# secup/ProjectUltra

Hardware: AMD Instinct MI355X
Metric: OFDM-1024 16QAM R3/4 frames decoded/sec (higher is better)
Workload: dtype f32

## Files before the change

projectultra_amd/csrc/demod_kernel.h:

```cpp
#ifndef ULTRA_DEMOD_KERNEL_H
#define ULTRA_DEMOD_KERNEL_H

#include <hip/hip_runtime.h>
#include <utility>
#include "device_types.h"
#include "pinned_math.h"
#include "phase_table.h"

namespace ultra_hip {
namespace dev {

constexpr int kWave = 64;
constexpr int kPhaseCap = 48;

__device__ __forceinline__ c32 mk(float re, float im) { c32 r; r.re = re; r.im = im; return r; }
__device__ __forceinline__ c32 cadd(c32 a, c32 b) { return mk(a.re + b.re, a.im + b.im); }
__device__ __forceinline__ c32 csub(c32 a, c32 b) { return mk(a.re - b.re, a.im - b.im); }
__device__ __forceinline__ c32 cconj(c32 a) { return mk(a.re, -a.im); }
__device__ __forceinline__ c32 cmul(c32 x, c32 y) {
    float ac = x.re * y.re, bd = x.im * y.im, ad = x.re * y.im, bc = x.im * y.re;
    return mk(ac - bd, ad + bc);
}
__device__ __forceinline__ c32 cdiv(c32 x, c32 y) {
    double a = x.re, b = x.im, c = y.re, d = y.im;
// ... 1346 lines not shown
    const LaneConst lc = lane_constants(D);
    for (int frame = blockIdx.x; frame < n_frames; frame += gridDim.x) {
        float* st = state + (size_t)frame * kStFloats;
        Track tr;
        load_track(st, tr);
        const bool presynced_loop = D.presynced && !synced_loop;
        const bool scalar_pilot_half = D.n_pilot == 0 && !presynced_loop;
        const bool compact = compact_pilot_state(D);
        if (!compact) sh.H[lane] = reinterpret_cast<const c32*>(st + kStH)[lane];
        else if (lane < D.n_pilot) sh.H[lc.pilot_slot] = reinterpret_cast<const c32*>(st + kStHp)[lane];
        c32 dprev = D.differential ? reinterpret_cast<const c32*>(st + kStDprev)[lane] : mk(1.0f, 0.0f);
        const bool adaptive = D.adaptive_eq != 0 && !D.differential;
        AdaptiveEq ad;
        ad.w = mk(1.0f, 0.0f); ad.P = 1.0f;
        if (adaptive) { ad.w = reinterpret_cast<const c32*>(st + kStLms)[lane]; ad.P = st[kStRlsP + lane]; }
        wave_sync();
        float dprev_abs = -1.0f;
        const bool tc_is_fixed = D.differential && D.n_pilot == 0 && n_sym_batch > 1;
        c32 tc0 = mk(1.0f, 0.0f);
        if (tc_is_fixed) tc0 = cexpj_bounded(timing_phase_of(lc.data_k, tr.timing, D.log2_fft));
        for (int ds = 0; ds < n_sym_batch; ++ds) {
            const c32* fq = fq_all + ((size_t)ds * n_frames + frame) * (2 * D.fq_half);
            if (scalar_pilot_half) { tr.ppc = mk(1.0f, 0.0f); tr.has_prev = 0; tr.snr_symbol_count++; }
            if (!presynced_loop || D.n_pilot != 0) {
                finish_channel_estimate(sh, D, lc, tr);
                if (adaptive && tr.snr_symbol_count - 1 < 3 && lane < D.n_data) ad.w = sh.H[lc.data_slot];
            }
            equalize_demap<MOD>(sh, D, lc, tr, dprev, fq,
                                llr + (size_t)frame * llr_stride + (size_t)(data_sym + ds) * D.llrs_per_symbol,
                                &dprev_abs, tc_is_fixed ? &tc0 : nullptr, nullptr, adaptive ? &ad : nullptr,
                                EQ ? eq_out + (size_t)frame * eq_stride + (size_t)ds * kMaxCarriers : nullptr);
            wave_sync();
        }
        if (!compact) reinterpret_cast<c32*>(st + kStH)[lane] = sh.H[lane];
        else if (lane < ((D.n_pilot + 15) & ~15))
            reinterpret_cast<c32*>(st + kStHp)[lane] = (lane < D.n_pilot) ? sh.H[lc.pilot_slot] : mk(0.0f, 0.0f);
        if (D.differential) reinterpret_cast<c32*>(st + kStDprev)[lane] = dprev;
        if (adaptive) { reinterpret_cast<c32*>(st + kStLms)[lane] = ad.w; st[kStRlsP + lane] = ad.P; }
        if (lane == 0) {
            st[st_ppc_re] = tr.ppc.re; st[st_ppc_im] = tr.ppc.im;
            st[st_flags] = (float)(tr.cpc_init | (tr.has_prev << 1) | (tr.has_dprev << 2));
            if (scalar_pilot_half) st[st_count] = (float)tr.snr_symbol_count;
            if (state_out) {
                float* so = state_out + (size_t)frame * ULTRA_HIP_STATE_FLOATS;
                so[ULTRA_HIP_STATE_FREQ_OFFSET_HZ] = tr.freq_offset_hz;
                so[ULTRA_HIP_STATE_NOISE_VARIANCE] = tr.noise_variance;
                so[ULTRA_HIP_STATE_SNR_LINEAR] = tr.snr_linear;
                so[ULTRA_HIP_STATE_TIMING_OFFSET] = tr.timing;
                so[ULTRA_HIP_STATE_CFO_PHASE] = tr.cfo_phase;
                so[ULTRA_HIP_STATE_MIXER_PHASE] = D.mixer_phase_end;
                so[ULTRA_HIP_STATE_SYMBOLS] = (float)tr.snr_symbol_count;
                so[ULTRA_HIP_STATE_RESERVED] = 0.0f;
            }
        }
        wave_sync();
    }
}

template <int MOD>
__global__ __launch_bounds__(kWave, 6) void track_diff_pair_kernel(
    const DemodConst* __restrict__ Dp, int n_frames, int data_sym, float* __restrict__ state,
    const c32* __restrict__ fq_all, float* __restrict__ llr, size_t llr_stride, float* __restrict__ state_out,
    int n_sym_batch) {
    static_assert(MOD == ULTRA_MOD_DBPSK || MOD == ULTRA_MOD_DQPSK || MOD == ULTRA_MOD_D8PSK, "differential layouts");
    constexpr int kBits = (MOD == ULTRA_MOD_DBPSK) ? 1 : (MOD == ULTRA_MOD_DQPSK) ? 2 : 3;
    const DemodConst& D = *Dp;
    const int lane = threadIdx.x, g = lane >> 5, sub = lane & 31;
    const bool is_data = sub < D.n_data;
    const int dsl = is_data ? D.data_slot[sub] : 0;
    const int data_fq = fq_index(D, D.bin[dsl]), data_k = D.k_of[dsl];
    const unsigned long long half_mask = g ? 0xffffffff00000000ull : 0x00000000ffffffffull;
    const int n_pairs = (n_frames + 1) / 2;
    for (int pair = blockIdx.x; pair < n_pairs; pair += gridDim.x) {
        const bool live = 2 * pair + g < n_frames;
        const int frame = live ? 2 * pair + g : n_frames - 1;
        float* st = state + (size_t)frame * kStFloats;
        Track tr;
        load_track(st, tr);
        c32 H = reinterpret_cast<const c32*>(st + kStH)[dsl];
        c32 dprev = reinterpret_cast<const c32*>(st + kStDprev)[sub];
        if (!tr.has_dprev) dprev = mk(1.0f, 0.0f);
        float prev_abs = cabs_(dprev);
        const c32 tc = cexpj_bounded(timing_phase_of(data_k, tr.timing, D.log2_fft));
        for (int ds = 0; ds < n_sym_batch; ++ds) {
            const c32* fq = fq_all + ((size_t)ds * n_frames + frame) * (2 * D.fq_half);
            tr.ppc = mk(1.0f, 0.0f); tr.has_prev = 0; tr.snr_symbol_count++;
            c32 eq = mk(0.0f, 0.0f);
            float nv = 100.0f;
            if (is_data) {
                const c32 received = fq[data_fq];
                const float h_power = cnorm(H);
                if (h_power > 1e-6f) {
                    const c32 t = cdivf(cmul(received, cconj(H)), h_power);
                    eq = cmul(cmul(t, tr.ppc), tc);
                    nv = tr.noise_variance / h_power;
                } else {
                    eq = cmul(cmul(received, tr.ppc), tc);
                    nv = 100.0f;
                }
                nv = fmax_std(1e-6f, fmin_std(100.0f, nv));
            }
            const float eq_abs = cabs_(eq);
            if (is_data) {
                float out[kBits];
                demap_carrier<MOD>(eq, dprev, nv * D.ce_margin, out, eq_abs, prev_abs);
                if (live) {
                    float* dst = llr + (size_t)frame * llr_stride + (size_t)(data_sym + ds) * D.llrs_per_symbol + sub * kBits;
#pragma unroll
                    for (int b = 0; b < kBits; ++b) dst[b] = out[b];
                }
                dprev = eq;
                prev_abs = eq_abs;
            }
            if ((MOD == ULTRA_MOD_DQPSK || MOD == ULTRA_MOD_D8PSK) && tr.snr_symbol_count >= 1) {
                bool strong = false;
                if (is_data) {
                    const float a = eq_abs;
                    strong = (a * a) > 0.1f;
                    if (strong) H = cmul(H, mk(1.0f, -0.0f));
                }
                const int valid = __popcll(__ballot(strong) & half_mask);
                if (valid >= 5) {
                    c32 p = cmul(cscale(tr.ppc, 1.0f), mk(1.0f, -0.0f));
                    const float mag = cabs_(p);
                    if (mag > 0.01f) p = cdivf(p, mag);
                    tr.ppc = p;
                }
            }
            tr.has_dprev = 1;
        }
        if (live && is_data) {
            reinterpret_cast<c32*>(st + kStH)[dsl] = H;
            reinterpret_cast<c32*>(st + kStDprev)[sub] = dprev;
        }
        if (live && sub == 0) {
            st[st_ppc_re] = tr.ppc.re; st[st_ppc_im] = tr.ppc.im;
            st[st_flags] = (float)(tr.cpc_init | (tr.has_prev << 1) | (tr.has_dprev << 2));
            st[st_count] = (float)tr.snr_symbol_count;
            if (state_out) {
                float* so = state_out + (size_t)frame * ULTRA_HIP_STATE_FLOATS;
                so[ULTRA_HIP_STATE_FREQ_OFFSET_HZ] = tr.freq_offset_hz;
                so[ULTRA_HIP_STATE_NOISE_VARIANCE] = tr.noise_variance;
                so[ULTRA_HIP_STATE_SNR_LINEAR] = tr.snr_linear;
                so[ULTRA_HIP_STATE_TIMING_OFFSET] = tr.timing;
                so[ULTRA_HIP_STATE_CFO_PHASE] = tr.cfo_phase;
                so[ULTRA_HIP_STATE_MIXER_PHASE] = D.mixer_phase_end;
                so[ULTRA_HIP_STATE_SYMBOLS] = (float)tr.snr_symbol_count;
                so[ULTRA_HIP_STATE_RESERVED] = 0.0f;
            }
        }
    }
}

template <int MOD>
__global__ __launch_bounds__(kWave, 6) void track_all_kernel(const DemodConst* __restrict__ Dp, int n_frames, int sym0, int n_sym_batch,
                                                             const float* __restrict__ trk_rec, const c32* __restrict__ fq_all,
                                                             float* __restrict__ llr, size_t llr_stride, float* __restrict__ state_out,
                                                             const float* __restrict__ state) {
    __shared__ TrackShared sh;
    const DemodConst& D = *Dp;
    const int lane = threadIdx.x;
    const LaneConst lc = lane_constants(D);
    const int total = n_frames * n_sym_batch;
    const int rec_floats = trk_rec_floats(D.n_pilot), rec_hp = trk_rec_hp(D.n_pilot);
    const int rec_mask = (D.n_pilot <= kTrkRecCompactPilots) ? 1 : 7;
    float nx_rec = 0.0f;
    c32 nx_hp = mk(0.0f, 0.0f), nx_fq = mk(0.0f, 0.0f);
    auto request = [&](int w) {
        const float* rec = trk_rec + (size_t)w * rec_floats;
        nx_rec = rec[lane & rec_mask];
        if (lane < D.n_pilot) nx_hp = reinterpret_cast<const c32*>(rec + rec_hp)[lane];
        if (lane < D.n_data) nx_fq = fq_all[(size_t)w * (2 * D.fq_half) + lc.data_fq];
    };
    if ((int)blockIdx.x < total) request((int)blockIdx.x);
    for (int w = blockIdx.x; w < total; w += gridDim.x) {
        const int frame = w % n_frames, ds = w / n_frames;
        Track tr;
        const float my_rec = nx_rec;
        const c32 my_hp = nx_hp, my_fq = nx_fq;
        if (w + (int)gridDim.x < total) request(w + (int)gridDim.x);
        tr.noise_variance = __int_as_float(__builtin_amdgcn_readlane(__float_as_int(my_rec), tk_noise));
        tr.timing = __int_as_float(__builtin_amdgcn_readlane(__float_as_int(my_rec), tk_timing));
        tr.ppc = mk(1.0f, 0.0f); tr.cpc = mk(1.0f, 0.0f);
        tr.cpc_init = 1; tr.has_prev = 1; tr.has_dprev = 0; tr.snr_symbol_count = 0; tr.symbols_since_sync = 0;
        if (lane < D.n_pilot) sh.H[lc.pilot_slot] = my_hp;
        c32 dprev = mk(1.0f, 0.0f);
        wave_sync();
        finish_channel_estimate(sh, D, lc, tr);
        equalize_demap<MOD>(sh, D, lc, tr, dprev, fq_all + (size_t)w * (2 * D.fq_half),
                            llr + (size_t)frame * llr_stride + (size_t)(sym0 + ds) * D.llrs_per_symbol, nullptr, nullptr, &my_fq);
        if (state_out && lane == 0 && ds == n_sym_batch - 1) {
            const float* st = state + (size_t)frame * kStFloats;
            float* so = state_out + (size_t)frame * ULTRA_HIP_STATE_FLOATS;
            so[ULTRA_HIP_STATE_FREQ_OFFSET_HZ] = st[st_cfo];
            so[ULTRA_HIP_STATE_NOISE_VARIANCE] = st[st_noise];
            so[ULTRA_HIP_STATE_SNR_LINEAR] = st[st_snr];
            so[ULTRA_HIP_STATE_TIMING_OFFSET] = st[st_timing];
            so[ULTRA_HIP_STATE_CFO_PHASE] = st[st_cfo_phase];
            so[ULTRA_HIP_STATE_MIXER_PHASE] = D.mixer_phase_end;
            so[ULTRA_HIP_STATE_SYMBOLS] = st[st_count];
            so[ULTRA_HIP_STATE_RESERVED] = 0.0f;
        }
        wave_sync();
    }
}

}
}
#endif
```

projectultra_amd/csrc/ultra_hip.hip:

```cpp
#include <hip/hip_runtime.h>

#include <dlfcn.h>
#include <cmath>
#include <cstdio>
#include <cstdlib>
#include <cstring>
#include <new>
#include <atomic>
#include <chrono>
#include <vector>

#include "../../include/ultra_hip.h"
#include "device_types.h"
#include "host_tables.h"
#include "demod_kernel.h"
#include "ldpc_kernel.h"
#include "ldpc_screen_kernel.h"
#include "ldpc_totals_kernel.h"
#include "acquire_kernel.h"
#include "stimulus_kernel.h"
#include "chirp_kernel.h"
#include "frame_kernel.h"

using namespace ultra_hip;
// ... 155 lines not shown
}
int ensure_list_workspace(ultra_hip_ctx* ctx, size_t n_cw) {
    if (ctx->ws_list_cw >= n_cw) return ULTRA_HIP_OK;
    if (ctx->d_ws_list) { UH_HIP(uh_stream_sync(ctx->stream)); (void)hipFree(ctx->d_ws_list); ctx->d_ws_list = nullptr; }
    ctx->ws_list_cw = 0;
    UH_HIP(hipMalloc(&ctx->d_ws_list, n_cw * sizeof(unsigned)));
    ctx->ws_list_cw = n_cw;
    return ULTRA_HIP_OK;
}
int ensure_llr_workspace(ultra_hip_ctx* ctx, size_t n_frames) {
    if (ctx->ws_llr_frames >= n_frames) return ULTRA_HIP_OK;
    if (ctx->d_ws_llr) { UH_HIP(uh_stream_sync(ctx->stream)); (void)hipFree(ctx->d_ws_llr); ctx->d_ws_llr = nullptr; }
    ctx->ws_llr_frames = 0;
    UH_HIP(hipMalloc(&ctx->d_ws_llr, n_frames * (size_t)ctx->geo.llrs_per_frame * sizeof(float)));
    ctx->ws_llr_frames = n_frames;
    return ULTRA_HIP_OK;
}

int launch_demod(ultra_hip_ctx* ctx, const float* d_audio, size_t frame_stride, const float* d_cfo_hz,
                 const float* d_cfo_phase, size_t n_frames, float* d_llr, size_t llr_stride, float* d_state,
                 const unsigned* d_frame_offset = nullptr, int sym_begin = 0, int sym_count = -1, c32* d_eq = nullptr) {
    if (n_frames == 0) return ULTRA_HIP_OK;
    const DemodConst& D = ctx->h_demod;
    const int s_begin = sym_begin, s_end = (sym_count < 0) ? D.n_train + D.n_data_sym : sym_begin + sym_count;
    if (s_begin < 0 || s_end > D.n_train + D.n_data_sym || s_end <= s_begin) return ULTRA_HIP_ERR_INVALID_ARG;
    if (s_begin > 0 && ctx->ws_demod_frames < n_frames) return ULTRA_HIP_ERR_INVALID_ARG;
    const int start_mode = (s_begin == 0 && sym_count >= 0) ? ctx->stream_start_mode : ULTRA_STREAM_START_FRESH;
    const float* start_timing = (start_mode == ULTRA_STREAM_START_TIMING) ? ctx->stream_start_timing : nullptr;
    if (s_begin == 0 && sym_count >= 0) { ctx->stream_start_mode = ULTRA_STREAM_START_FRESH; ctx->stream_start_timing = nullptr; }
    if (start_mode == ULTRA_STREAM_START_SYNC && (ctx->ws_demod_frames < n_frames || D.presynced)) return ULTRA_HIP_ERR_INVALID_ARG;
    const bool cfo_given = (s_begin == 0) ? (d_cfo_hz != nullptr || start_mode != ULTRA_STREAM_START_FRESH) : ctx->stream_cfo_given;
    if (s_begin == 0) ctx->stream_cfo_given = cfo_given;
    { const int rc_ws = ensure_demod_workspace(ctx, n_frames); if (rc_ws != ULTRA_HIP_OK) return rc_ws; }
    auto mix_grid = [&](size_t items) {
        size_t per_cu = ctx->mix_wg_per_cu > 0 ? (size_t)ctx->mix_wg_per_cu
                                               : std::min<size_t>(128, std::max<size_t>(24, items / ((size_t)ctx->cu_count * 24)));
        return (unsigned)std::min(items, (size_t)ctx->cu_count * per_cu);
    };
    const unsigned grid_fft = mix_grid(n_frames);
    const unsigned grid_trk = (unsigned)std::min(n_frames, (size_t)ctx->cu_count * 128);
    hipStream_t st = ctx->stream;
    if (D.log2_fft != 10 && D.log2_fft != 9) return ULTRA_HIP_ERR_UNSUPPORTED;
    const int n_sym = s_end - s_begin;
    const bool cfo_is_zero = !D.presynced && D.n_pilot == 0 && !cfo_given;
    const unsigned* seg_tab = cfo_is_zero ? nullptr : ctx->d_ws_seg;
    bool all_symbols_at_once = cfo_is_zero && n_sym > 1 && n_frames * (size_t)n_sym < 0x7fffffffull;
    bool deferred = !ctx->old_chain && !d_eq && !D.differential && D.n_pilot > 0 && D.n_pilot <= dev::kPwPilots && D.n_train == 0 &&
                    !D.presynced && D.adaptive_eq == 0 && n_frames * (size_t)n_sym < 0x7fffffffull;
    const size_t fold_rows = n_frames * (size_t)n_sym;
    auto over_limit = [&](size_t bytes) { return ctx->ws_limit_bytes != 0 && bytes > ctx->ws_limit_bytes; };
    if ((all_symbols_at_once || deferred) &&
        (over_limit(fold_rows * (size_t)(2 * D.fq_half) * sizeof(c32)) || ensure_fq_workspace(ctx, fold_rows) != ULTRA_HIP_OK)) {
        (void)hipGetLastError();
        all_symbols_at_once = false; deferred = false;
        ctx->status_flags |= ULTRA_HIP_ST_DEMOD_WORKSPACE_FALLBACK;
    }
    if (deferred && (over_limit(fold_rows * (size_t)dev::trk_rec_floats(D.n_pilot) * sizeof(float)) || ensure_trk_workspace(ctx, fold_rows) != ULTRA_HIP_OK)) {
        (void)hipGetLastError(); deferred = false;
        ctx->status_flags |= ULTRA_HIP_ST_DEMOD_WORKSPACE_FALLBACK;
    }
    { const int rc_fq = ensure_fq_workspace(ctx, n_frames); if (rc_fq != ULTRA_HIP_OK) return rc_fq; }
    const bool fresh_pilot = deferred && s_begin == 0 && !cfo_given;
    const int synced_loop = (D.presynced && s_begin > 0) ? 1 : 0;
    if (s_begin == 0 && start_mode == ULTRA_STREAM_START_SYNC) {
        LaunchSpan span(ctx, ULTRA_HIP_K_INIT_STATE);
        hipLaunchKernelGGL(dev::resync_state_kernel, dim3(grid_trk), dim3(dev::kWave), 0, st, d_cfo_hz, d_cfo_phase, (int)n_frames, ctx->d_ws_state,
                           (!D.differential || D.n_pilot > 0) ? 1 : 0);
    } else if (s_begin == 0 && !fresh_pilot) {
        LaunchSpan span(ctx, ULTRA_HIP_K_INIT_STATE);
        const int compact = (!D.differential && D.n_pilot > 0 && D.n_train == 0) ? 1 : 0;
        hipLaunchKernelGGL(dev::init_state_kernel, dim3(grid_trk), dim3(dev::kWave), 0, st, d_cfo_hz, d_cfo_phase,
                           (int)n_frames, ctx->d_ws_state, compact, (D.adaptive_eq != 0 && !D.differential) ? 1 : 0, start_timing);
    }
    if (s_begin == 0 && D.presynced && d_cfo_hz) {
        LaunchSpan span(ctx, ULTRA_HIP_K_INIT_STATE);
        hipLaunchKernelGGL(dev::train_cfo_kernel, dim3((unsigned)((n_frames + 255) / 256)), dim3(256), 0, st, ctx->d_demod, ctx->d_nco,
                           d_audio, frame_stride, d_frame_offset, d_cfo_hz, (int)n_frames, ctx->d_ws_state);
    }
    auto launch_mix = [&](unsigned g, int sym, c32* fq, const unsigned* tab, int n_sym_batch) {
        auto go = [&](auto kernel, unsigned threads) {
            hipLaunchKernelGGL(kernel, dim3(g), dim3(threads), 0, st, ctx->d_demod, ctx->d_nco, ctx->d_twiddle, d_audio, frame_stride,
                               d_frame_offset, (int)n_frames, sym, fq, tab, n_sym_batch);
        };
        if (tab && n_sym_batch != 1) return (int)ULTRA_HIP_ERR_UNSUPPORTED;
        if (D.log2_fft == 10) {
            if (tab) go(dev::mix_fft2_kernel<10, true>, 2 * dev::kWave);
            else go(dev::mix_fft2_kernel<10, false>, 2 * dev::kWave);
        } else {
            if (tab) go(dev::mix_fft2_kernel<9, true>, dev::kWave);
            else go(dev::mix_fft2_kernel<9, false>, dev::kWave);
        }
        return (int)ULTRA_HIP_OK;
    };
    if (all_symbols_at_once) {
        LaunchSpan span(ctx, ULTRA_HIP_K_MIX_FFT, n_frames * (unsigned long long)n_sym);
        const unsigned g = mix_grid(n_frames * (size_t)n_sym);
        const int rc_mix = launch_mix(g, s_begin, ctx->d_ws_fq, nullptr, n_sym);
        if (rc_mix != ULTRA_HIP_OK) return rc_mix;
    }
    int mixed_upto = 0;
    for (int s = s_begin; s < s_end; ++s) {
        c32* fq_s = ctx->d_ws_fq + ((all_symbols_at_once || deferred) ? (size_t)(s - s_begin) * n_frames * (size_t)(2 * D.fq_half) : (size_t)0);
        float* rec_s = deferred ? ctx->d_ws_trk + (size_t)(s - s_begin) * n_frames * dev::trk_rec_floats(D.n_pilot) : nullptr;
        const bool first_at_zero = s <= 1 && !D.presynced && !cfo_given;
        const unsigned* seg_tab_s = first_at_zero ? nullptr : seg_tab;
        if (!cfo_is_zero && !first_at_zero) {
            LaunchSpan span(ctx, ULTRA_HIP_K_WALK, n_frames);
            hipLaunchKernelGGL(dev::cfo_walk_kernel, dim3((unsigned)((n_frames + 255) / 256)), dim3(256), 0, st, ctx->d_demod,
                               (int)n_frames, ctx->d_ws_state, ctx->d_ws_seg);
        }
        if (!all_symbols_at_once && s >= mixed_upto) {
            const bool two = deferred && s == 0 && first_at_zero && s + 1 < s_end && n_frames * (size_t)2 < 0x7fffffffull;
            LaunchSpan span(ctx, seg_tab_s ? ULTRA_HIP_K_MIX_FFT_ROT : ULTRA_HIP_K_MIX_FFT, n_frames * (two ? 2ull : 1ull));
            int rc_mix;
            if (two) {
                rc_mix = launch_mix(mix_grid(n_frames * 2), s, fq_s, nullptr, 2);
                mixed_upto = 2;
            } else {
                rc_mix = launch_mix(grid_fft, s, fq_s, seg_tab_s, 1);
            }
            if (rc_mix != ULTRA_HIP_OK) return rc_mix;
        }
        const bool training = s < D.n_train;
        const bool last = (s == s_end - 1);
        if (training) {
            LaunchSpan span(ctx, ULTRA_HIP_K_TRACK, n_frames);
            hipLaunchKernelGGL(dev::train_kernel, dim3(grid_trk), dim3(dev::kWave), 0, st, ctx->d_demod, (int)n_frames, s,
                               ctx->d_ws_state, fq_s);
            continue;
        }
        if (D.n_pilot != 0) {
            LaunchSpan span(ctx, ULTRA_HIP_K_PILOT, n_frames);
            if (D.n_pilot <= 16) {
                const unsigned g = (unsigned)std::min((n_frames + 3) / 4, (size_t)ctx->cu_count * 256);
                if (fresh_pilot && s == 0)
                    hipLaunchKernelGGL((dev::track_pilot_kernel<16, true>), dim3(g), dim3(dev::kWave), 0, st, ctx->d_demod, (int)n_frames,
                                       ctx->d_ws_state, fq_s, rec_s);
                else
                    hipLaunchKernelGGL((dev::track_pilot_kernel<16, false>), dim3(g), dim3(dev::kWave), 0, st, ctx->d_demod, (int)n_frames,
                                       ctx->d_ws_state, fq_s, rec_s);
            } else {
                const unsigned g = (unsigned)std::min((n_frames + 1) / 2, (size_t)ctx->cu_count * 512);
                if (fresh_pilot && s == 0)
                    hipLaunchKernelGGL((dev::track_pilot_kernel<32, true>), dim3(g), dim3(dev::kWave), 0, st, ctx->d_demod, (int)n_frames,
                                       ctx->d_ws_state, fq_s, rec_s);
                else
                    hipLaunchKernelGGL((dev::track_pilot_kernel<32, false>), dim3(g), dim3(dev::kWave), 0, st, ctx->d_demod, (int)n_frames,
                                       ctx->d_ws_state, fq_s, rec_s);
            }
        }
        if (deferred) {
            if (!last) continue;
            LaunchSpan span(ctx, ULTRA_HIP_K_TRACK, n_frames * (unsigned long long)n_sym);
            const unsigned g = (unsigned)std::min(n_frames * (size_t)n_sym, (size_t)ctx->cu_count * 128);
#define UH_TRACK_ALL(MOD)                                                                                                  \
    hipLaunchKernelGGL(dev::track_all_kernel<MOD>, dim3(g), dim3(dev::kWave), 0, st, ctx->d_demod, (int)n_frames, s_begin, n_sym, \
                       ctx->d_ws_trk, ctx->d_ws_fq, d_llr, llr_stride, d_state, ctx->d_ws_state)
            switch (D.modulation) {
                case ULTRA_MOD_BPSK: UH_TRACK_ALL(ULTRA_MOD_BPSK); break;
                case ULTRA_MOD_QPSK: UH_TRACK_ALL(ULTRA_MOD_QPSK); break;
                case ULTRA_MOD_QAM16: UH_TRACK_ALL(ULTRA_MOD_QAM16); break;
                case ULTRA_MOD_QAM32: UH_TRACK_ALL(ULTRA_MOD_QAM32); break;
                case ULTRA_MOD_QAM64: UH_TRACK_ALL(ULTRA_MOD_QAM64); break;
                case ULTRA_MOD_QAM256: UH_TRACK_ALL(ULTRA_MOD_QAM256); break;
                default: return ULTRA_HIP_ERR_UNSUPPORTED;
            }
#undef UH_TRACK_ALL
            break;
        }
        const int track_batch = all_symbols_at_once ? s_end - s : 1;
        const bool last_launch = last || all_symbols_at_once;
#define UH_TRACK(MOD)                                                                                            \
    do {                                                                                                         \
        if (d_eq)                                                                                                \
            hipLaunchKernelGGL((dev::track_kernel<MOD, true>), dim3(grid_trk), dim3(dev::kWave), 0, st, ctx->d_demod, (int)n_frames, \
                               s - D.n_train, ctx->d_ws_state, fq_s, d_llr, llr_stride, last_launch ? d_state : nullptr, track_batch, \
                               synced_loop, d_eq + (size_t)(s - std::max(s_begin, (int)D.n_train)) * kMaxCarriers, eq_stride);        \
        else                                                                                                     \
            hipLaunchKernelGGL((dev::track_kernel<MOD, false>), dim3(grid_trk), dim3(dev::kWave), 0, st, ctx->d_demod, (int)n_frames, \
                               s - D.n_train, ctx->d_ws_state, fq_s, d_llr, llr_stride, last_launch ? d_state : nullptr, track_batch, \
                               synced_loop, (c32*)nullptr, (size_t)0);                                           \
    } while (0)
        LaunchSpan span(ctx, ULTRA_HIP_K_TRACK, n_frames * (unsigned long long)track_batch);
        const size_t eq_stride = (size_t)(s_end - std::max(s_begin, (int)D.n_train)) * kMaxCarriers;
        const bool pair_frames = !ctx->old_chain && !d_eq && D.differential && D.n_pilot == 0 && !D.presynced && D.n_carriers <= 32 &&
                                 D.n_train == 0;
#define UH_TRACK_PAIR(MOD)                                                                                                         \
    hipLaunchKernelGGL(dev::track_diff_pair_kernel<MOD>, dim3((unsigned)std::min((n_frames + 1) / 2, (size_t)ctx->cu_count * 128)),  \
                       dim3(dev::kWave), 0, st, ctx->d_demod, (int)n_frames, s - D.n_train, ctx->d_ws_state, fq_s, d_llr, llr_stride, \
                       last_launch ? d_state : nullptr, track_batch)
        if (pair_frames && D.modulation == ULTRA_MOD_DBPSK) UH_TRACK_PAIR(ULTRA_MOD_DBPSK);
        else if (pair_frames && D.modulation == ULTRA_MOD_DQPSK) UH_TRACK_PAIR(ULTRA_MOD_DQPSK);
        else if (pair_frames && D.modulation == ULTRA_MOD_D8PSK) UH_TRACK_PAIR(ULTRA_MOD_D8PSK);
        else
#undef UH_TRACK_PAIR
        switch (D.modulation) {
            case ULTRA_MOD_DBPSK: UH_TRACK(ULTRA_MOD_DBPSK); break;
            case ULTRA_MOD_BPSK: UH_TRACK(ULTRA_MOD_BPSK); break;
            case ULTRA_MOD_DQPSK: UH_TRACK(ULTRA_MOD_DQPSK); break;
            case ULTRA_MOD_QPSK: UH_TRACK(ULTRA_MOD_QPSK); break;
            case ULTRA_MOD_D8PSK: UH_TRACK(ULTRA_MOD_D8PSK); break;
            case ULTRA_MOD_QAM16: UH_TRACK(ULTRA_MOD_QAM16); break;
            case ULTRA_MOD_QAM32: UH_TRACK(ULTRA_MOD_QAM32); break;
            case ULTRA_MOD_QAM64: UH_TRACK(ULTRA_MOD_QAM64); break;
            case ULTRA_MOD_QAM256: UH_TRACK(ULTRA_MOD_QAM256); break;
            default: return ULTRA_HIP_ERR_UNSUPPORTED;
        }
#undef UH_TRACK
        if (all_symbols_at_once) break;
    }
    UH_HIP(hipGetLastError());
    return ULTRA_HIP_OK;
}

int launch_ldpc(ultra_hip_ctx* ctx, const float* d_llr, size_t llr_stride, size_t n_cw, uint8_t* d_bytes,
                int32_t* d_iters, uint8_t* d_ok, float* d_llr_total, int block_len = 0, int block_stride = 0) {
    if (n_cw == 0) return ULTRA_HIP_OK;
    const LdpcPlan& P = ctx->h_plan;
    unsigned int* counter = ctx->d_work + (size_t)(ctx->work_slot++ & 15) * dev::kLdpcQueueWords;
    UH_HIP(hipMemsetAsync(counter, 0, dev::kLdpcQueueWords * sizeof(unsigned int), ctx->stream));
    if (ctx->h_tplan.valid) {
        const LdpcTPlan& T = ctx->h_tplan;
        const size_t tlds = (size_t)T.lds_bytes;
        if (T.t_pad != T.var_rounds * 256 || T.r_base != T.t_pad + 128 || T.r_pad != T.r_base + T.n_planes * 256 ||
            T.stage_v != T.r_pad + 128 || T.stage_p != T.stage_v + T.var_rounds * 256 ||
            T.lds_bytes != T.stage_v + ldpc_stage_bytes(T.var_rounds, T.row_rounds))
            return ULTRA_HIP_ERR_UNSUPPORTED;
#define UH_TOTALS_LAUNCH(RR, VR, RP, VP, WV, CP)                                                                  \
    do {                                                                                                          \
        const size_t lds_wg = (CP) ? (size_t)T.stage_v + 4 * (size_t)(T.n_checked + T.m) : tlds;                  \
        const size_t per_cu = std::max<size_t>(1, std::min<size_t>(4 * (WV), (size_t)(160 * 1024) / lds_wg));     \
        const unsigned grid = (unsigned)std::min(n_cw, (size_t)ctx->cu_count * per_cu);                           \
        if (d_llr_total)                                                                                          \
            hipLaunchKernelGGL((dev::ldpc_totals_kernel<RR, VR, RP, VP, true, WV, false>), dim3(grid), dim3(dev::kLdpcThreads), tlds, \
                               ctx->stream, ctx->d_tplan, d_llr, llr_stride, (int)n_cw, d_bytes, d_iters, d_ok,   \
                               d_llr_total, counter, (int)ctx->deint_step, ctx->d_deint_table, block_len, block_stride, \
                               (const unsigned*)nullptr, 0u);                                                     \
        else                                                                                                      \
            hipLaunchKernelGGL((dev::ldpc_totals_kernel<RR, VR, RP, VP, false, WV, CP>), dim3(grid), dim3(dev::kLdpcThreads), lds_wg, \
                               ctx->stream, ctx->d_tplan, d_llr, llr_stride, (int)n_cw, d_bytes, d_iters, d_ok,   \
                               d_llr_total, counter, (int)ctx->deint_step, ctx->d_deint_table, block_len, block_stride, \
                               (const unsigned*)work_list, gate);                                                 \
    } while (0)
        auto is = [&](int rr, int vr, unsigned long long rp, unsigned long long vp) {
            return T.row_rounds == rr && T.var_rounds == vr && T.row_prof == rp && T.var_prof == vp;
        };
        const bool r34 = is(3, 6, 0x666ull, 0x333333ull), r56 = is(2, 4, 0x66ull, 0x3333ull), r23 = is(4, 7, 0x6666ull, 0x3333333ull),
                   r14 = is(8, 3, kPlaceRowProf_R1_4, kPlaceVarProf_R1_4), r13 = is(6, 6, kPlaceRowProf_R1_3, kPlaceVarProf_R1_3),
                   r12 = is(6, 6, kPlaceRowProf_R1_2, kPlaceVarProf_R1_2);
        const bool launched = r34 || r56 || r23 || r14 || r13 || r12;
        if (launched) {
            LaunchSpan span(ctx, ULTRA_HIP_K_LDPC, n_cw);
            unsigned* work_list = nullptr;
            unsigned gate = 0u;
            const bool screen = ctx->screen_mode != 0 && ctx->d_screen_pos && T.max_iterations > 0 && !d_llr_total &&
                                (ctx->screen_mode == 2 || n_cw >= kScreenMinCodewords) && n_cw <= 0x7fffffffull;
            if (screen && ensure_list_workspace(ctx, n_cw) != ULTRA_HIP_OK) {
                (void)hipGetLastError();
                ctx->status_flags |= ULTRA_HIP_ST_SCREEN_LIST_UNAVAILABLE;
            } else if (screen) {
                if (ctx->screen_pos_stale) {
                    hipLaunchKernelGGL(dev::ldpc_screen_prepare_kernel, dim3(1), dim3(512), 0, ctx->stream, ctx->d_screen_var, T.m, T.k,
                                       (int)ctx->deint_step, ctx->d_deint_table, ctx->d_screen_pos);
                    ctx->screen_pos_stale = false;
                }
                const int sample_n = (int)std::min<size_t>(n_cw, (size_t)dev::kScreenSampleMax);
                const int sample_stride = (int)(n_cw / (size_t)sample_n);
                gate = ctx->screen_mode == 2 ? 0u : (unsigned)((sample_n + 2) / 3);
                work_list = ctx->d_ws_list;
                const unsigned gs = (unsigned)((sample_n + dev::kScreenWaves - 1) / dev::kScreenWaves);
                const unsigned gf = (unsigned)((n_cw + dev::kScreenChunk - 1) / dev::kScreenChunk);
#define UH_SCREEN_LAUNCH(RR, EP)                                                                                                 \
    do {                                                                                                                         \
        hipLaunchKernelGGL((dev::ldpc_screen_kernel<RR, EP, true>), dim3(gs), dim3(dev::kScreenThreads), 0, ctx->stream, ctx->d_screen_pos, \
                           d_llr, llr_stride, (int)n_cw, block_len, block_stride, T.decoded_bytes, d_bytes, d_iters, d_ok, counter,     \
                           work_list, gate, sample_n, sample_stride);                                                            \
        hipLaunchKernelGGL((dev::ldpc_screen_kernel<RR, EP, false>), dim3(gf), dim3(dev::kScreenThreads), 0, ctx->stream, ctx->d_screen_pos, \
                           d_llr, llr_stride, (int)n_cw, block_len, block_stride, T.decoded_bytes, d_bytes, d_iters, d_ok, counter,     \
                           work_list, gate, sample_n, sample_stride);                                                            \
    } while (0)
                const unsigned long long ep = ctx->screen_prof;
                switch (T.row_rounds) {
                    case 2: UH_SCREEN_LAUNCH(2, 0x77ull); break;
                    case 3: UH_SCREEN_LAUNCH(3, 0x777ull); break;
                    case 4: UH_SCREEN_LAUNCH(4, 0x7777ull); break;
                    case 6: if (ep == 0x244677ull) UH_SCREEN_LAUNCH(6, 0x244677ull);
                            else if (ep == 0x235677ull) UH_SCREEN_LAUNCH(6, 0x235677ull);
                            else UH_SCREEN_LAUNCH(6, 0x777777ull);
                            break;
                    case 8: if (ep == 0x33456677ull) UH_SCREEN_LAUNCH(8, 0x33456677ull);
                            else UH_SCREEN_LAUNCH(8, 0x77777777ull);
                            break;
                    default: work_list = nullptr; break;
                }
#undef UH_SCREEN_LAUNCH
                if (work_list) { ++ctx->screen_launches; ctx->last_screen_gate = gate; ctx->last_screen_sample_n = (uint32_t)sample_n; }
            }
            const bool compact = r34 && !d_llr_total && ctx->deint_step == 1u && !ctx->d_deint_table && T.k == 486 && T.n_checked == 325 &&
                                 T.m == 162;
            if (r34 && compact) UH_TOTALS_LAUNCH(3, 6, 0x666ull, 0x333333ull, 5, true);
            else if (r34) UH_TOTALS_LAUNCH(3, 6, 0x666ull, 0x333333ull, 5, false);
            else if (r56) UH_TOTALS_LAUNCH(2, 4, 0x66ull, 0x3333ull, 6, false);
            else if (r23) UH_TOTALS_LAUNCH(4, 7, 0x6666ull, 0x3333333ull, 4, false);
            else if (r14) UH_TOTALS_LAUNCH(8, 3, kPlaceRowProf_R1_4, kPlaceVarProf_R1_4, 3, false);
            else if (r13) UH_TOTALS_LAUNCH(6, 6, kPlaceRowProf_R1_3, kPlaceVarProf_R1_3, 4, false);
            else UH_TOTALS_LAUNCH(6, 6, kPlaceRowProf_R1_2, kPlaceVarProf_R1_2, 4, false);
            if (work_list) (void)hipMemcpyAsync(ctx->d_status, counter, 4 * sizeof(unsigned), hipMemcpyDeviceToDevice, ctx->stream);
// ... 1214 lines not shown
```

Baseline: 55.48 million.

## Deepen track_all prefetch queue and assign frames per workgroup

Each workgroup in track_all_kernel now owns whole frames and walks all their symbols in turn, instead of striding over a flat frame*symbol index. The one-deep register prefetch becomes a ring of four outstanding loads to hide more global memory latency. Grid size is now capped by frame count rather than frame*symbols. Loads become unconditional, clamped to index 0 when out of range, which adds register pressure and some wasted fetches. Parallelism also drops when there are few frames.

```diff
diff --git a/projectultra_amd/csrc/demod_kernel.h b/projectultra_amd/csrc/demod_kernel.h
--- a/projectultra_amd/csrc/demod_kernel.h
+++ b/projectultra_amd/csrc/demod_kernel.h
@@ -1522,8 +1522,15 @@
     }
 }
 
+#ifndef UH_TRK_ALL_AHEAD
+#define UH_TRK_ALL_AHEAD 4
+#endif
+#ifndef UH_TRK_ALL_WAVES
+#define UH_TRK_ALL_WAVES 6
+#endif
+constexpr int kTrkAllAhead = UH_TRK_ALL_AHEAD;
 template <int MOD>
-__global__ __launch_bounds__(kWave, 6) void track_all_kernel(const DemodConst* __restrict__ Dp, int n_frames, int sym0, int n_sym_batch,
+__global__ __launch_bounds__(kWave, UH_TRK_ALL_WAVES) void track_all_kernel(const DemodConst* __restrict__ Dp, int n_frames, int sym0, int n_sym_batch,
                                                              const float* __restrict__ trk_rec, const c32* __restrict__ fq_all,
                                                              float* __restrict__ llr, size_t llr_stride, float* __restrict__ state_out,
                                                              const float* __restrict__ state) {
@@ -1531,47 +1538,57 @@
     const DemodConst& D = *Dp;
     const int lane = threadIdx.x;
     const LaneConst lc = lane_constants(D);
-    const int total = n_frames * n_sym_batch;
     const int rec_floats = trk_rec_floats(D.n_pilot), rec_hp = trk_rec_hp(D.n_pilot);
     const int rec_mask = (D.n_pilot <= kTrkRecCompactPilots) ? 1 : 7;
-    float nx_rec = 0.0f;
-    c32 nx_hp = mk(0.0f, 0.0f), nx_fq = mk(0.0f, 0.0f);
-    auto request = [&](int w) {
+    float q_rec[kTrkAllAhead];
+    c32 q_hp[kTrkAllAhead], q_fq[kTrkAllAhead];
+    int r_frame = blockIdx.x, r_s = 0;
+    auto request = [&](float& rec_o, c32& hp_o, c32& fq_o) {
+        const int w = (r_frame < n_frames) ? r_s * n_frames + r_frame : 0;
         const float* rec = trk_rec + (size_t)w * rec_floats;
-        nx_rec = rec[lane & rec_mask];
-        if (lane < D.n_pilot) nx_hp = reinterpret_cast<const c32*>(rec + rec_hp)[lane];
-        if (lane < D.n_data) nx_fq = fq_all[(size_t)w * (2 * D.fq_half) + lc.data_fq];
+        rec_o = rec[lane & rec_mask];
+        hp_o = reinterpret_cast<const c32*>(rec + rec_hp)[(lane < D.n_pilot) ? lane : 0];
+        fq_o = fq_all[(size_t)w * (2 * D.fq_half) + lc.data_fq];
+        if (++r_s == n_sym_batch) { r_s = 0; r_frame += gridDim.x; }
     };
-    if ((int)blockIdx.x < total) request((int)blockIdx.x);
-    for (int w = blockIdx.x; w < total; w += gridDim.x) {
-        const int frame = w % n_frames, ds = w / n_frames;
-        Track tr;
-        const float my_rec = nx_rec;
-        const c32 my_hp = nx_hp, my_fq = nx_fq;
-        if (w + (int)gridDim.x < total) request(w + (int)gridDim.x);
-        tr.noise_variance = __int_as_float(__builtin_amdgcn_readlane(__float_as_int(my_rec), tk_noise));
-        tr.timing = __int_as_float(__builtin_amdgcn_readlane(__float_as_int(my_rec), tk_timing));
-        tr.ppc = mk(1.0f, 0.0f); tr.cpc = mk(1.0f, 0.0f);
-        tr.cpc_init = 1; tr.has_prev = 1; tr.has_dprev = 0; tr.snr_symbol_count = 0; tr.symbols_since_sync = 0;
-        if (lane < D.n_pilot) sh.H[lc.pilot_slot] = my_hp;
-        c32 dprev = mk(1.0f, 0.0f);
-        wave_sync();
-        finish_channel_estimate(sh, D, lc, tr);
-        equalize_demap<MOD>(sh, D, lc, tr, dprev, fq_all + (size_t)w * (2 * D.fq_half),
-                            llr + (size_t)frame * llr_stride + (size_t)(sym0 + ds) * D.llrs_per_symbol, nullptr, nullptr, &my_fq);
-        if (state_out && lane == 0 && ds == n_sym_batch - 1) {
-            const float* st = state + (size_t)frame * kStFloats;
-            float* so = state_out + (size_t)frame * ULTRA_HIP_STATE_FLOATS;
-            so[ULTRA_HIP_STATE_FREQ_OFFSET_HZ] = st[st_cfo];
-            so[ULTRA_HIP_STATE_NOISE_VARIANCE] = st[st_noise];
-            so[ULTRA_HIP_STATE_SNR_LINEAR] = st[st_snr];
-            so[ULTRA_HIP_STATE_TIMING_OFFSET] = st[st_timing];
-            so[ULTRA_HIP_STATE_CFO_PHASE] = st[st_cfo_phase];
-            so[ULTRA_HIP_STATE_MIXER_PHASE] = D.mixer_phase_end;
-            so[ULTRA_HIP_STATE_SYMBOLS] = st[st_count];
-            so[ULTRA_HIP_STATE_RESERVED] = 0.0f;
-        }
-        wave_sync();
+#pragma unroll
+    for (int u = 0; u < kTrkAllAhead; ++u) {
+        request(q_rec[u], q_hp[u], q_fq[u]);
+    }
+    int frame = blockIdx.x, ds = 0;
+    while (frame < n_frames) {
+#pragma unroll
+        for (int u = 0; u < kTrkAllAhead; ++u) {
+            if (frame < n_frames) {
+                const int w = ds * n_frames + frame;
+                Track tr;
+                tr.noise_variance = __int_as_float(__builtin_amdgcn_readlane(__float_as_int(q_rec[u]), tk_noise));
+                tr.timing = __int_as_float(__builtin_amdgcn_readlane(__float_as_int(q_rec[u]), tk_timing));
+                tr.ppc = mk(1.0f, 0.0f); tr.cpc = mk(1.0f, 0.0f);
+                tr.cpc_init = 1; tr.has_prev = 1; tr.has_dprev = 0; tr.snr_symbol_count = 0; tr.symbols_since_sync = 0;
+                if (lane < D.n_pilot) sh.H[lc.pilot_slot] = q_hp[u];
+                c32 dprev = mk(1.0f, 0.0f);
+                wave_sync();
+                finish_channel_estimate(sh, D, lc, tr);
+                equalize_demap<MOD>(sh, D, lc, tr, dprev, fq_all + (size_t)w * (2 * D.fq_half),
+                                    llr + (size_t)frame * llr_stride + (size_t)(sym0 + ds) * D.llrs_per_symbol, nullptr, nullptr, &q_fq[u]);
+                if (state_out && lane == 0 && ds == n_sym_batch - 1) {
+                    const float* st = state + (size_t)frame * kStFloats;
+                    float* so = state_out + (size_t)frame * ULTRA_HIP_STATE_FLOATS;
+                    so[ULTRA_HIP_STATE_FREQ_OFFSET_HZ] = st[st_cfo];
+                    so[ULTRA_HIP_STATE_NOISE_VARIANCE] = st[st_noise];
+                    so[ULTRA_HIP_STATE_SNR_LINEAR] = st[st_snr];
+                    so[ULTRA_HIP_STATE_TIMING_OFFSET] = st[st_timing];
+                    so[ULTRA_HIP_STATE_CFO_PHASE] = st[st_cfo_phase];
+                    so[ULTRA_HIP_STATE_MIXER_PHASE] = D.mixer_phase_end;
+                    so[ULTRA_HIP_STATE_SYMBOLS] = st[st_count];
+                    so[ULTRA_HIP_STATE_RESERVED] = 0.0f;
+                }
+                wave_sync();
+                if (++ds == n_sym_batch) { ds = 0; frame += gridDim.x; }
+            }
+            request(q_rec[u], q_hp[u], q_fq[u]);
+        }
     }
 }
 
diff --git a/projectultra_amd/csrc/ultra_hip.hip b/projectultra_amd/csrc/ultra_hip.hip
--- a/projectultra_amd/csrc/ultra_hip.hip
+++ b/projectultra_amd/csrc/ultra_hip.hip
@@ -331,7 +331,10 @@
         if (deferred) {
             if (!last) continue;
             LaunchSpan span(ctx, ULTRA_HIP_K_TRACK, n_frames * (unsigned long long)n_sym);
-            const unsigned g = (unsigned)std::min(n_frames * (size_t)n_sym, (size_t)ctx->cu_count * 128);
+#ifndef UH_TRK_ALL_WG_PER_CU
+#define UH_TRK_ALL_WG_PER_CU 128
+#endif
+            const unsigned g = (unsigned)std::min(n_frames, (size_t)ctx->cu_count * UH_TRK_ALL_WG_PER_CU);
 #define UH_TRACK_ALL(MOD)                                                                                                  \
     hipLaunchKernelGGL(dev::track_all_kernel<MOD>, dim3(g), dim3(dev::kWave), 0, st, ctx->d_demod, (int)n_frames, s_begin, n_sym, \
                        ctx->d_ws_trk, ctx->d_ws_fq, d_llr, llr_stride, d_state, ctx->d_ws_state)
```

After: 56.28 million, median of 6. +1.4%, better.
